# lifeiteng/vall-e

Measured on NVIDIA H100. Metric: audio tokens/sec (AR+NAR d=1024/12L), higher is better.
Workload: dtype bf16

## Files before the change

valle_b200/csrc/attention_wgmma.cu:

```cuda
#include <math_constants.h>

#include "common.cuh"
#include "kernels.cuh"
#include "sm90_ptx.cuh"

namespace vb {
namespace fa3 {

using namespace tc;

constexpr int HD = 64, BQ = 128, BKV = 64;
constexpr int kThreads = 288;
constexpr int kStages = 3;
constexpr int kBoxBytes = 64 * HD * 2;
constexpr int kQBytes = 2 * kBoxBytes;
constexpr int kStageBytes = 2 * kBoxBytes;
constexpr int kSmemBytes = kQBytes + kStages * kStageBytes + 1024  + 256 ;

__device__ __forceinline__ uint64_t make_smem_desc_mn(uint32_t smem_addr) {
  uint64_t d = 0;
  d |= (uint64_t)((smem_addr & 0x3FFFF) >> 4);
  d |= (uint64_t)(1024 >> 4) << 16;
  d |= (uint64_t)(1024 >> 4) << 32;
  d |= (uint64_t)1 << 62;
  return d;
}
__device__ __forceinline__ float ex2(float x) {
  float y;
  asm("ex2.approx.ftz.f32 %0, %1;" : "=f"(y) : "f"(x));
  return y;
}
__device__ __forceinline__ uint32_t pack_bf16(float lo, float hi) {
  __nv_bfloat162 p = __floats2bfloat162_rn(lo, hi);
  return *reinterpret_cast<uint32_t *>(&p);
}

__global__ void __launch_bounds__(kThreads, 2)
attn_wgmma_kernel(const __grid_constant__ CUtensorMap tmap_qkv, int n_head, const int32_t *__restrict__ cu_seqlens,
                  const int32_t *__restrict__ text_lens, const int32_t *__restrict__ seg1_lens, int seg1_start,
                  int mask_mode, bf16 *__restrict__ out, bf16 *__restrict__ kcache, bf16 *__restrict__ vcache,
                  int64_t cache_seq_stride, int cache_cap) {
  const int b = blockIdx.z, h = blockIdx.y;
  const int r0 = cu_seqlens[b], L = cu_seqlens[b + 1] - r0;
  const int q0 = blockIdx.x * BQ;
  if (q0 >= L) return;
  const int S = (mask_mode != VB_MASK_FULL) ? text_lens[b] : 0;
  const int c1 = (mask_mode >= VB_MASK_PADDED_AR) ? seg1_lens[b] : 0;
  const int d = n_head * HD;
  const int q_hi = min(q0 + BQ, L);
  const int kv_max = (mask_mode == VB_MASK_VALLE_AR) ? max(S, q_hi) : L;
  const int n_tiles = (kv_max + BKV - 1) / BKV;

  extern __shared__ uint8_t smem_raw[];
  uint8_t *sq = reinterpret_cast<uint8_t *>((reinterpret_cast<uintptr_t>(smem_raw) + 1023) & ~(uintptr_t)1023);
  uint8_t *ring = sq + kQBytes;
  uint64_t *bars = reinterpret_cast<uint64_t *>(ring + kStages * kStageBytes);
  uint64_t *q_bar = bars, *full_bar = bars + 1, *empty_bar = bars + 1 + kStages;

  const int wg = threadIdx.x >> 7, t = threadIdx.x & 127, lane = threadIdx.x & 31;
  if (threadIdx.x == 0) {
    prefetch_tmap(&tmap_qkv);
    mbar_init(q_bar, 1);
    for (int i = 0; i < kStages; ++i) {
      mbar_init(&full_bar[i], 1);
      mbar_init(&empty_bar[i], 8);
    }
    asm volatile("fence.mbarrier_init.release.cluster;" ::: "memory");
  }
  __syncthreads();

  if (wg == 2) {
    if (t == 0) {
      mbar_expect_tx(q_bar, kQBytes);
      tma_load_2d(&tmap_qkv, q_bar, sq, h * HD, r0 + q0);
      tma_load_2d(&tmap_qkv, q_bar, sq + kBoxBytes, h * HD, r0 + q0 + 64);
      int stage = 0;
      uint32_t phase = 0;
      for (int it = 0; it < n_tiles; ++it) {
        mbar_wait(&empty_bar[stage], phase ^ 1);
        uint8_t *dst = ring + stage * kStageBytes;
        mbar_expect_tx(&full_bar[stage], kStageBytes);
        tma_load_2d(&tmap_qkv, &full_bar[stage], dst, d + h * HD, r0 + it * BKV);
        tma_load_2d(&tmap_qkv, &full_bar[stage], dst + kBoxBytes, 2 * d + h * HD, r0 + it * BKV);
        if (++stage == kStages) {
          stage = 0;
          phase ^= 1;
        }
      }
    }
    return;
  }

  const int half = wg;
  const int row_a = q0 + half * 64 + wg_row(t, 0), row_b = row_a + 8;
  const RowMask lim_a = make_row_mask(mask_mode, row_a, L, S, seg1_start, c1);
  const RowMask lim_b = make_row_mask(mask_mode, row_b, L, S, seg1_start, c1);
  const float sc = 0.125f * 1.4426950408889634f;
  const uint64_t qdesc = make_smem_desc(smem_u32(sq + half * kBoxBytes));

  float o[32];
#pragma unroll
  for (int i = 0; i < 32; ++i) o[i] = 0.f;
  float m_a = -CUDART_INF_F, m_b = -CUDART_INF_F, l_a = 0.f, l_b = 0.f;

  mbar_wait(q_bar, 0);
  int stage = 0;
  uint32_t phase = 0;
  for (int it = 0; it < n_tiles; ++it) {
    const int j0 = it * BKV;
    mbar_wait(&full_bar[stage], phase);
    uint8_t *sk = ring + stage * kStageBytes, *sv = sk + kBoxBytes;
    float s[32];
    const uint64_t kdesc = make_smem_desc(smem_u32(sk));
    wgmma_fence();
#pragma unroll
    for (int k = 0; k < HD / WGMMA_K; ++k) wgmma_m64n64k16(s, qdesc + (uint64_t)(k * 2), kdesc + (uint64_t)(k * 2), k != 0);
    wgmma_commit();
    wgmma_wait<0>();
    wgmma_fence_regs(s);
    if (kcache != nullptr && j0 == q0 + half * 64) {
#pragma unroll
      for (int i = 0; i < 4; ++i) {
        const int idx = t + i * 128;
        const int r = idx >> 3, c = idx & 7;
        if (j0 + r < L) {
          const int64_t off = (int64_t)b * cache_seq_stride + ((int64_t)h * cache_cap + j0 + r) * HD + c * 8;
          const int so = r * 128 + ((c ^ (r & 7)) << 4);
          *reinterpret_cast<uint4 *>(kcache + off) = *reinterpret_cast<const uint4 *>(sk + so);
          *reinterpret_cast<uint4 *>(vcache + off) = *reinterpret_cast<const uint4 *>(sv + so);
        }
      }
    }
    float mx_a = -CUDART_INF_F, mx_b = -CUDART_INF_F;
#pragma unroll
    for (int i = 0; i < 32; ++i) {
      const int c = j0 + wg_col(t, i);
      if ((i >> 1) & 1) {
        s[i] = lim_b.ok(c) ? s[i] * sc : -CUDART_INF_F;
        mx_b = fmaxf(mx_b, s[i]);
      } else {
        s[i] = lim_a.ok(c) ? s[i] * sc : -CUDART_INF_F;
        mx_a = fmaxf(mx_a, s[i]);
      }
    }
    mx_a = fmaxf(mx_a, __shfl_xor_sync(0xffffffffu, mx_a, 1));
    mx_a = fmaxf(mx_a, __shfl_xor_sync(0xffffffffu, mx_a, 2));
    mx_b = fmaxf(mx_b, __shfl_xor_sync(0xffffffffu, mx_b, 1));
    mx_b = fmaxf(mx_b, __shfl_xor_sync(0xffffffffu, mx_b, 2));
    const float mn_a = fmaxf(m_a, mx_a), mn_b = fmaxf(m_b, mx_b);
    const float mu_a = mn_a == -CUDART_INF_F ? 0.f : mn_a, mu_b = mn_b == -CUDART_INF_F ? 0.f : mn_b;
    const float corr_a = ex2(m_a - mu_a), corr_b = ex2(m_b - mu_b);
    m_a = mn_a;
    m_b = mn_b;
    float rs_a = 0.f, rs_b = 0.f;
#pragma unroll
    for (int i = 0; i < 32; ++i) {
      if ((i >> 1) & 1) {
        s[i] = ex2(s[i] - mu_b);
        rs_b += s[i];
        o[i] *= corr_b;
      } else {
        s[i] = ex2(s[i] - mu_a);
        rs_a += s[i];
        o[i] *= corr_a;
      }
    }
    l_a = l_a * corr_a + rs_a;
    l_b = l_b * corr_b + rs_b;
    uint32_t pa[4][4];
#pragma unroll
    for (int ks = 0; ks < 4; ++ks) {
      pa[ks][0] = pack_bf16(s[8 * ks + 0], s[8 * ks + 1]);
      pa[ks][1] = pack_bf16(s[8 * ks + 2], s[8 * ks + 3]);
      pa[ks][2] = pack_bf16(s[8 * ks + 4], s[8 * ks + 5]);
      pa[ks][3] = pack_bf16(s[8 * ks + 6], s[8 * ks + 7]);
    }
    const uint64_t vdesc = make_smem_desc_mn(smem_u32(sv));
    wgmma_fence();
#pragma unroll
    for (int ks = 0; ks < 4; ++ks) wgmma_m64n64k16_rs_tb(o, pa[ks], vdesc + (uint64_t)(ks * (16 * 128 >> 4)));
    wgmma_commit();
    wgmma_wait<0>();
    wgmma_fence_regs(o);
    __syncwarp();
    if (lane == 0) mbar_arrive(&empty_bar[stage]);
    if (++stage == kStages) {
      stage = 0;
      phase ^= 1;
    }
  }
  l_a += __shfl_xor_sync(0xffffffffu, l_a, 1);
  l_a += __shfl_xor_sync(0xffffffffu, l_a, 2);
  l_b += __shfl_xor_sync(0xffffffffu, l_b, 1);
  l_b += __shfl_xor_sync(0xffffffffu, l_b, 2);
  const float inv_a = 1.f / l_a, inv_b = 1.f / l_b;
#pragma unroll
  for (int i = 0; i < 32; i += 2) {
    const bool rb = (i >> 1) & 1;
    const int row = rb ? row_b : row_a;
    if (row >= L) continue;
    const float inv = rb ? inv_b : inv_a;
    *reinterpret_cast<uint32_t *>(out + (int64_t)(r0 + row) * d + h * HD + wg_col(t, i)) =
        pack_bf16(o[i] * inv, o[i + 1] * inv);
  }
}

}

int launch_attention_wgmma(const bf16 *qkv, int64_t M, int B, int n_head, const int32_t *cu_seqlens,
                           const int32_t *text_lens, const int32_t *seg1_lens, int seg1_start, int max_seqlen,
                           int mask_mode, bf16 *out, bf16 *kcache, bf16 *vcache, int64_t cache_seq_stride,
                           int cache_cap, cudaStream_t s) {
  if (M == 0 || B == 0) return VB_OK;
  VB_CHECK_ARG((reinterpret_cast<uintptr_t>(qkv) & 15) == 0, "wgmma attention: qkv must be 16-byte aligned");
  CUtensorMap tm;
  VB_TRY(tc::make_tmap(&tm, qkv, M, 3 * n_head * fa3::HD, 3 * (int64_t)n_head * fa3::HD, 64));
  static PerDeviceOnce once;
  if (once.first())
    VB_CUDA(cudaFuncSetAttribute(fa3::attn_wgmma_kernel, cudaFuncAttributeMaxDynamicSharedMemorySize, fa3::kSmemBytes));
  dim3 grid((max_seqlen + fa3::BQ - 1) / fa3::BQ, n_head, B);
  fa3::attn_wgmma_kernel<<<grid, fa3::kThreads, fa3::kSmemBytes, s>>>(tm, n_head, cu_seqlens, text_lens, seg1_lens,
                                                                      seg1_start, mask_mode, out, kcache, vcache,
                                                                      cache_seq_stride, cache_cap);
  VB_LAUNCH_CHECK();
  return VB_OK;
}

}
```

valle_b200/csrc/sm90_ptx.cuh:

```cuda
#pragma once
#include <cuda.h>

#include <mutex>

#include "common.cuh"

namespace vb {
namespace tc {

constexpr int BK = 64;
constexpr int WGMMA_K = 16;

__device__ __forceinline__ uint32_t smem_u32(const void *p) {
  return static_cast<uint32_t>(__cvta_generic_to_shared(p));
}
__device__ __forceinline__ void mbar_init(uint64_t *bar, uint32_t count) {
  asm volatile("mbarrier.init.shared::cta.b64 [%0], %1;" ::"r"(smem_u32(bar)), "r"(count));
}
__device__ __forceinline__ void mbar_expect_tx(uint64_t *bar, uint32_t bytes) {
  asm volatile("mbarrier.arrive.expect_tx.shared::cta.b64 _, [%0], %1;" ::"r"(smem_u32(bar)), "r"(bytes)
               : "memory");
}
__device__ __forceinline__ void mbar_arrive(uint64_t *bar) {
  asm volatile("mbarrier.arrive.shared::cta.b64 _, [%0];" ::"r"(smem_u32(bar)) : "memory");
}
__device__ __forceinline__ uint32_t mbar_try_wait(uint64_t *bar, uint32_t parity) {
  uint32_t ok;
  asm volatile(
      "{\n"
      ".reg .pred p;\n"
      "mbarrier.try_wait.parity.shared::cta.b64 p, [%1], %2;\n"
      "selp.u32 %0, 1, 0, p;\n"
      "}\n"
      : "=r"(ok)
      : "r"(smem_u32(bar)), "r"(parity)
      : "memory");
  return ok;
}
__device__ __forceinline__ void mbar_wait(uint64_t *bar, uint32_t parity) {
  while (!mbar_try_wait(bar, parity)) {
  }
}
__device__ __forceinline__ void tma_load_2d(const CUtensorMap *map, uint64_t *bar, void *dst, int c0, int c1) {
  asm volatile(
      "cp.async.bulk.tensor.2d.shared::cluster.global.tile.mbarrier::complete_tx::bytes [%0], [%1, {%3, %4}], [%2];"
      ::"r"(smem_u32(dst)), "l"(map), "r"(smem_u32(bar)), "r"(c0), "r"(c1)
      : "memory");
}
__device__ __forceinline__ void prefetch_tmap(const CUtensorMap *map) {
  asm volatile("prefetch.tensormap [%0];" ::"l"(map) : "memory");
}
__device__ __forceinline__ void wgmma_fence() { asm volatile("wgmma.fence.sync.aligned;" ::: "memory"); }
__device__ __forceinline__ void wgmma_commit() { asm volatile("wgmma.commit_group.sync.aligned;" ::: "memory"); }
template <int N> __device__ __forceinline__ void wgmma_wait() {
  asm volatile("wgmma.wait_group.sync.aligned %0;" ::"n"(N) : "memory");
}
template <int R> __device__ __forceinline__ void wgmma_fence_regs(float (&d)[R]) {
#pragma unroll
  for (int i = 0; i < R; ++i) asm volatile("" : "+f"(d[i])::"memory");
}
__device__ __forceinline__ uint64_t make_smem_desc(uint32_t smem_addr) {
  uint64_t d = 0;
  d |= (uint64_t)((smem_addr & 0x3FFFF) >> 4);
  d |= (uint64_t)1 << 16;
  d |= (uint64_t)(1024 >> 4) << 32;
  d |= (uint64_t)1 << 62;
  return d;
}
__device__ __forceinline__ int wg_row(int t, int i) { return ((t >> 5) << 4) + ((t & 31) >> 2) + (((i >> 1) & 1) << 3); }
__device__ __forceinline__ int wg_col(int t, int i) { return ((i >> 2) << 3) + ((t & 3) << 1) + (i & 1); }

__device__ __forceinline__ void wgmma_m64n64k16(float (&d)[32], uint64_t adesc, uint64_t bdesc, uint32_t accumulate) {
  asm volatile(
      "{\n"
      ".reg .pred p;\n"
      "setp.ne.b32 p, %34, 0;\n"
      "wgmma.mma_async.sync.aligned.m64n64k16.f32.bf16.bf16 "
      "{%0, %1, %2, %3, %4, %5, %6, %7, %8, %9, %10, %11, %12, %13, %14, %15, %16, %17, %18, %19, %20, %21, %22, %23, %24, %25, %26, %27, %28, %29, %30, %31}, "
      "%32, %33, p, 1, 1, 0, 0;\n"
      "}\n"
      : "+f"(d[0]), "+f"(d[1]), "+f"(d[2]), "+f"(d[3]), "+f"(d[4]), "+f"(d[5]), "+f"(d[6]), "+f"(d[7]), "+f"(d[8]), "+f"(d[9]), "+f"(d[10]), "+f"(d[11]), "+f"(d[12]), "+f"(d[13]), "+f"(d[14]), "+f"(d[15]), "+f"(d[16]), "+f"(d[17]), "+f"(d[18]), "+f"(d[19]), "+f"(d[20]), "+f"(d[21]), "+f"(d[22]), "+f"(d[23]), "+f"(d[24]), "+f"(d[25]), "+f"(d[26]), "+f"(d[27]), "+f"(d[28]), "+f"(d[29]), "+f"(d[30]), "+f"(d[31])
      : "l"(adesc), "l"(bdesc), "r"(accumulate));
}

__device__ __forceinline__ void wgmma_m64n128k16(float (&d)[64], uint64_t adesc, uint64_t bdesc, uint32_t accumulate) {
  asm volatile(
      "{\n"
      ".reg .pred p;\n"
      "setp.ne.b32 p, %66, 0;\n"
      "wgmma.mma_async.sync.aligned.m64n128k16.f32.bf16.bf16 "
      "{%0, %1, %2, %3, %4, %5, %6, %7, %8, %9, %10, %11, %12, %13, %14, %15, %16, %17, %18, %19, %20, %21, %22, %23, %24, %25, %26, %27, %28, %29, %30, %31, %32, %33, %34, %35, %36, %37, %38, %39, %40, %41, %42, %43, %44, %45, %46, %47, %48, %49, %50, %51, %52, %53, %54, %55, %56, %57, %58, %59, %60, %61, %62, %63}, "
      "%64, %65, p, 1, 1, 0, 0;\n"
      "}\n"
      : "+f"(d[0]), "+f"(d[1]), "+f"(d[2]), "+f"(d[3]), "+f"(d[4]), "+f"(d[5]), "+f"(d[6]), "+f"(d[7]), "+f"(d[8]), "+f"(d[9]), "+f"(d[10]), "+f"(d[11]), "+f"(d[12]), "+f"(d[13]), "+f"(d[14]), "+f"(d[15]), "+f"(d[16]), "+f"(d[17]), "+f"(d[18]), "+f"(d[19]), "+f"(d[20]), "+f"(d[21]), "+f"(d[22]), "+f"(d[23]), "+f"(d[24]), "+f"(d[25]), "+f"(d[26]), "+f"(d[27]), "+f"(d[28]), "+f"(d[29]), "+f"(d[30]), "+f"(d[31]), "+f"(d[32]), "+f"(d[33]), "+f"(d[34]), "+f"(d[35]), "+f"(d[36]), "+f"(d[37]), "+f"(d[38]), "+f"(d[39]), "+f"(d[40]), "+f"(d[41]), "+f"(d[42]), "+f"(d[43]), "+f"(d[44]), "+f"(d[45]), "+f"(d[46]), "+f"(d[47]), "+f"(d[48]), "+f"(d[49]), "+f"(d[50]), "+f"(d[51]), "+f"(d[52]), "+f"(d[53]), "+f"(d[54]), "+f"(d[55]), "+f"(d[56]), "+f"(d[57]), "+f"(d[58]), "+f"(d[59]), "+f"(d[60]), "+f"(d[61]), "+f"(d[62]), "+f"(d[63])
      : "l"(adesc), "l"(bdesc), "r"(accumulate));
}

__device__ __forceinline__ void wgmma_m64n64k16_rs_tb(float (&d)[32], const uint32_t (&a)[4], uint64_t bdesc) {
  asm volatile(
      "{\n"
      ".reg .pred p;\n"
      "setp.ne.b32 p, %37, 0;\n"
      "wgmma.mma_async.sync.aligned.m64n64k16.f32.bf16.bf16 "
      "{%0, %1, %2, %3, %4, %5, %6, %7, %8, %9, %10, %11, %12, %13, %14, %15, %16, %17, %18, %19, %20, %21, %22, %23, %24, %25, %26, %27, %28, %29, %30, %31}, "
      "{%32, %33, %34, %35}, %36, p, 1, 1, 1;\n"
      "}\n"
      : "+f"(d[0]), "+f"(d[1]), "+f"(d[2]), "+f"(d[3]), "+f"(d[4]), "+f"(d[5]), "+f"(d[6]), "+f"(d[7]), "+f"(d[8]), "+f"(d[9]), "+f"(d[10]), "+f"(d[11]), "+f"(d[12]), "+f"(d[13]), "+f"(d[14]), "+f"(d[15]), "+f"(d[16]), "+f"(d[17]), "+f"(d[18]), "+f"(d[19]), "+f"(d[20]), "+f"(d[21]), "+f"(d[22]), "+f"(d[23]), "+f"(d[24]), "+f"(d[25]), "+f"(d[26]), "+f"(d[27]), "+f"(d[28]), "+f"(d[29]), "+f"(d[30]), "+f"(d[31])
      : "r"(a[0]), "r"(a[1]), "r"(a[2]), "r"(a[3]), "l"(bdesc), "r"(1));
}

typedef CUresult (*EncodeTiledFn)(CUtensorMap *, CUtensorMapDataType, cuuint32_t, void *, const cuuint64_t *,
                                  const cuuint64_t *, const cuuint32_t *, const cuuint32_t *,
                                  CUtensorMapInterleave, CUtensorMapSwizzle, CUtensorMapL2promotion,
                                  CUtensorMapFloatOOBfill);

inline EncodeTiledFn get_encode() {
  static EncodeTiledFn fn = nullptr;
  static std::once_flag once;
  std::call_once(once, [] {
    void *p = nullptr;
    cudaDriverEntryPointQueryResult q;
    if (cudaGetDriverEntryPoint("cuTensorMapEncodeTiled", &p, cudaEnableDefault, &q) == cudaSuccess &&
        q == cudaDriverEntryPointSuccess)
      fn = reinterpret_cast<EncodeTiledFn>(p);
  });
  return fn;
}

inline int make_tmap_f32_dense(CUtensorMap *map, const void *ptr, int64_t rows, int64_t cols, int64_t ld, int box_rows,
                               int box_cols) {
  EncodeTiledFn enc = get_encode();
  if (!enc) {
    set_error("tensor map: cuTensorMapEncodeTiled entry point unavailable");
    return VB_ERR_CUDA;
  }
  cuuint64_t dims[2] = {(cuuint64_t)cols, (cuuint64_t)rows};
  cuuint64_t strides[1] = {(cuuint64_t)ld * 4};
  cuuint32_t box[2] = {(cuuint32_t)box_cols, (cuuint32_t)box_rows};
  cuuint32_t estr[2] = {1, 1};
  CUresult r = enc(map, CU_TENSOR_MAP_DATA_TYPE_FLOAT32, 2, const_cast<void *>(ptr), dims, strides, box, estr,
                   CU_TENSOR_MAP_INTERLEAVE_NONE, CU_TENSOR_MAP_SWIZZLE_NONE, CU_TENSOR_MAP_L2_PROMOTION_L2_256B,
                   CU_TENSOR_MAP_FLOAT_OOB_FILL_NONE);
  if (r != CUDA_SUCCESS) {
    set_error("tensor map: cuTensorMapEncodeTiled (fp32 dense) failed (%d) rows=%lld cols=%lld ld=%lld", (int)r,
              (long long)rows, (long long)cols, (long long)ld);
    return VB_ERR_CUDA;
  }
  return VB_OK;
}
inline int make_tmap(CUtensorMap *map, const void *ptr, int64_t rows, int K, int64_t ld, int box_rows) {
  EncodeTiledFn enc = get_encode();
  if (!enc) {
    set_error("wgmma gemm: cuTensorMapEncodeTiled entry point unavailable");
    return VB_ERR_CUDA;
  }
  cuuint64_t dims[2] = {(cuuint64_t)K, (cuuint64_t)rows};
  cuuint64_t strides[1] = {(cuuint64_t)ld * 2};
  cuuint32_t box[2] = {(cuuint32_t)BK, (cuuint32_t)box_rows};
  cuuint32_t estr[2] = {1, 1};
  CUresult r = enc(map, CU_TENSOR_MAP_DATA_TYPE_BFLOAT16, 2, const_cast<void *>(ptr), dims, strides, box, estr,
                   CU_TENSOR_MAP_INTERLEAVE_NONE, CU_TENSOR_MAP_SWIZZLE_128B, CU_TENSOR_MAP_L2_PROMOTION_L2_256B,
                   CU_TENSOR_MAP_FLOAT_OOB_FILL_NONE);
  if (r != CUDA_SUCCESS) {
    set_error("wgmma gemm: cuTensorMapEncodeTiled failed (%d) rows=%lld K=%d ld=%lld", (int)r, (long long)rows, K,
              (long long)ld);
    return VB_ERR_CUDA;
  }
  return VB_OK;
}

}
}
```

Measured before the change: 296,700.

## Restructure FA3 attention kernel with 3 consumer warpgroups and QK/PV overlap

Moves the producer to warpgroup 0 and uses three consumer warpgroups (BQ=192) with setmaxnreg register reallocation, one CTA per SM, and four pipeline stages. It software-pipelines the loop so the next tile's QK^T wgmma is issued alongside the previous tile's PV wgmma, overlapping softmax with tensor-core work. It also skips per-element mask evaluation for tiles that are fully visible. The trade-offs are lower CTA occupancy, larger Q tiles that waste work on short sequences, and more complex barrier and register fencing logic.

```diff
diff --git a/valle_b200/csrc/attention_wgmma.cu b/valle_b200/csrc/attention_wgmma.cu
--- a/valle_b200/csrc/attention_wgmma.cu
+++ b/valle_b200/csrc/attention_wgmma.cu
@@ -9,12 +9,16 @@
 
 using namespace tc;
 
-constexpr int HD = 64, BQ = 128, BKV = 64;
-constexpr int kThreads = 288;
-constexpr int kStages = 3;
+constexpr int HD = 64, BKV = 64;
 constexpr int kBoxBytes = 64 * HD * 2;
-constexpr int kQBytes = 2 * kBoxBytes;
 constexpr int kStageBytes = 2 * kBoxBytes;
+
+constexpr int NWG = 3;
+constexpr int BQ = 64 * NWG;
+constexpr int kThreads = 128 * (NWG + 1);
+constexpr int kStages = 4;
+constexpr int kProdRegs = 24, kConsRegs = 160;
+constexpr int kQBytes = NWG * kBoxBytes;
 constexpr int kSmemBytes = kQBytes + kStages * kStageBytes + 1024  + 256 ;
 
 __device__ __forceinline__ uint64_t make_smem_desc_mn(uint32_t smem_addr) {
@@ -34,8 +38,67 @@
   __nv_bfloat162 p = __floats2bfloat162_rn(lo, hi);
   return *reinterpret_cast<uint32_t *>(&p);
 }
-
-__global__ void __launch_bounds__(kThreads, 2)
+template <int R> __device__ __forceinline__ void fence_u32(uint32_t (&a)[R][4]) {
+#pragma unroll
+  for (int i = 0; i < R; ++i)
+#pragma unroll
+    for (int k = 0; k < 4; ++k) asm volatile("" : "+r"(a[i][k])::"memory");
+}
+
+__device__ __forceinline__ void issue_qk(float (&s)[32], uint64_t qdesc, const uint8_t *sk) {
+  const uint64_t kdesc = make_smem_desc(smem_u32(sk));
+#pragma unroll
+  for (int k = 0; k < HD / WGMMA_K; ++k) wgmma_m64n64k16(s, qdesc + (uint64_t)(k * 2), kdesc + (uint64_t)(k * 2), k != 0);
+}
+__device__ __forceinline__ void issue_pv(float (&o)[32], const uint32_t (&pa)[4][4], const uint8_t *sv) {
+  const uint64_t vdesc = make_smem_desc_mn(smem_u32(sv));
+#pragma unroll
+  for (int ks = 0; ks < 4; ++ks) wgmma_m64n64k16_rs_tb(o, pa[ks], vdesc + (uint64_t)(ks * (16 * 128 >> 4)));
+}
+
+template <bool MASKED>
+__device__ __forceinline__ void softmax_block(float (&s)[32], int j0, int t, const RowMask &lim_a, const RowMask &lim_b,
+                                              float &m_a, float &m_b, float &l_a, float &l_b, float &corr_a,
+                                              float &corr_b) {
+  const float sc = 0.125f * 1.4426950408889634f;
+  float mx_a = -CUDART_INF_F, mx_b = -CUDART_INF_F;
+#pragma unroll
+  for (int i = 0; i < 32; ++i) {
+    const int c = j0 + wg_col(t, i);
+    if ((i >> 1) & 1) {
+      s[i] = (!MASKED || lim_b.ok(c)) ? __fmul_rn(s[i], sc) : -CUDART_INF_F;
+      mx_b = fmaxf(mx_b, s[i]);
+    } else {
+      s[i] = (!MASKED || lim_a.ok(c)) ? __fmul_rn(s[i], sc) : -CUDART_INF_F;
+      mx_a = fmaxf(mx_a, s[i]);
+    }
+  }
+  mx_a = fmaxf(mx_a, __shfl_xor_sync(0xffffffffu, mx_a, 1));
+  mx_a = fmaxf(mx_a, __shfl_xor_sync(0xffffffffu, mx_a, 2));
+  mx_b = fmaxf(mx_b, __shfl_xor_sync(0xffffffffu, mx_b, 1));
+  mx_b = fmaxf(mx_b, __shfl_xor_sync(0xffffffffu, mx_b, 2));
+  const float mn_a = fmaxf(m_a, mx_a), mn_b = fmaxf(m_b, mx_b);
+  const float mu_a = mn_a == -CUDART_INF_F ? 0.f : mn_a, mu_b = mn_b == -CUDART_INF_F ? 0.f : mn_b;
+  corr_a = ex2(m_a - mu_a);
+  corr_b = ex2(m_b - mu_b);
+  m_a = mn_a;
+  m_b = mn_b;
+  float rs_a = 0.f, rs_b = 0.f;
+#pragma unroll
+  for (int i = 0; i < 32; ++i) {
+    if ((i >> 1) & 1) {
+      s[i] = ex2(s[i] - mu_b);
+      rs_b += s[i];
+    } else {
+      s[i] = ex2(s[i] - mu_a);
+      rs_a += s[i];
+    }
+  }
+  l_a = l_a * corr_a + rs_a;
+  l_b = l_b * corr_b + rs_b;
+}
+
+__global__ void __launch_bounds__(kThreads, 1)
 attn_wgmma_kernel(const __grid_constant__ CUtensorMap tmap_qkv, int n_head, const int32_t *__restrict__ cu_seqlens,
                   const int32_t *__restrict__ text_lens, const int32_t *__restrict__ seg1_lens, int seg1_start,
                   int mask_mode, bf16 *__restrict__ out, bf16 *__restrict__ kcache, bf16 *__restrict__ vcache,
@@ -44,6 +107,7 @@
   const int r0 = cu_seqlens[b], L = cu_seqlens[b + 1] - r0;
   const int q0 = blockIdx.x * BQ;
   if (q0 >= L) return;
+  const int n_wg = min(NWG, (L - q0 + 63) >> 6);
   const int S = (mask_mode != VB_MASK_FULL) ? text_lens[b] : 0;
   const int c1 = (mask_mode >= VB_MASK_PADDED_AR) ? seg1_lens[b] : 0;
   const int d = n_head * HD;
@@ -63,17 +127,17 @@
     mbar_init(q_bar, 1);
     for (int i = 0; i < kStages; ++i) {
       mbar_init(&full_bar[i], 1);
-      mbar_init(&empty_bar[i], 8);
+      mbar_init(&empty_bar[i], 4 * n_wg);
     }
     asm volatile("fence.mbarrier_init.release.cluster;" ::: "memory");
   }
   __syncthreads();
 
-  if (wg == 2) {
+  if (wg == 0) {
+    setmaxnreg_dec<kProdRegs>();
     if (t == 0) {
-      mbar_expect_tx(q_bar, kQBytes);
-      tma_load_2d(&tmap_qkv, q_bar, sq, h * HD, r0 + q0);
-      tma_load_2d(&tmap_qkv, q_bar, sq + kBoxBytes, h * HD, r0 + q0 + 64);
+      mbar_expect_tx(q_bar, n_wg * kBoxBytes);
+      for (int w = 0; w < n_wg; ++w) tma_load_2d(&tmap_qkv, q_bar, sq + w * kBoxBytes, h * HD, r0 + q0 + 64 * w);
       int stage = 0;
       uint32_t phase = 0;
       for (int it = 0; it < n_tiles; ++it) {
@@ -90,35 +154,25 @@
     }
     return;
   }
-
-  const int half = wg;
-  const int row_a = q0 + half * 64 + wg_row(t, 0), row_b = row_a + 8;
+  setmaxnreg_inc<kConsRegs>();
+
+  const int w = wg - 1;
+  if (w >= n_wg) return;
+  const int row_a = q0 + w * 64 + wg_row(t, 0), row_b = row_a + 8;
   const RowMask lim_a = make_row_mask(mask_mode, row_a, L, S, seg1_start, c1);
   const RowMask lim_b = make_row_mask(mask_mode, row_b, L, S, seg1_start, c1);
-  const float sc = 0.125f * 1.4426950408889634f;
-  const uint64_t qdesc = make_smem_desc(smem_u32(sq + half * kBoxBytes));
+  const uint64_t qdesc = make_smem_desc(smem_u32(sq + w * kBoxBytes));
 
   float o[32];
 #pragma unroll
   for (int i = 0; i < 32; ++i) o[i] = 0.f;
   float m_a = -CUDART_INF_F, m_b = -CUDART_INF_F, l_a = 0.f, l_b = 0.f;
-
-  mbar_wait(q_bar, 0);
-  int stage = 0;
-  uint32_t phase = 0;
-  for (int it = 0; it < n_tiles; ++it) {
-    const int j0 = it * BKV;
-    mbar_wait(&full_bar[stage], phase);
-    uint8_t *sk = ring + stage * kStageBytes, *sv = sk + kBoxBytes;
-    float s[32];
-    const uint64_t kdesc = make_smem_desc(smem_u32(sk));
-    wgmma_fence();
-#pragma unroll
-    for (int k = 0; k < HD / WGMMA_K; ++k) wgmma_m64n64k16(s, qdesc + (uint64_t)(k * 2), kdesc + (uint64_t)(k * 2), k != 0);
-    wgmma_commit();
-    wgmma_wait<0>();
-    wgmma_fence_regs(s);
-    if (kcache != nullptr && j0 == q0 + half * 64) {
+  float s[32];
+  uint32_t pa[4][4];
+
+  auto softmax_step = [&](int j0, const uint8_t *sk, float &corr_a, float &corr_b) {
+    if (kcache != nullptr && j0 == q0 + w * 64) {
+      const uint8_t *sv = sk + kBoxBytes;
 #pragma unroll
       for (int i = 0; i < 4; ++i) {
         const int idx = t + i * 128;
@@ -131,43 +185,16 @@
         }
       }
     }
-    float mx_a = -CUDART_INF_F, mx_b = -CUDART_INF_F;
-#pragma unroll
-    for (int i = 0; i < 32; ++i) {
-      const int c = j0 + wg_col(t, i);
-      if ((i >> 1) & 1) {
-        s[i] = lim_b.ok(c) ? s[i] * sc : -CUDART_INF_F;
-        mx_b = fmaxf(mx_b, s[i]);
-      } else {
-        s[i] = lim_a.ok(c) ? s[i] * sc : -CUDART_INF_F;
-        mx_a = fmaxf(mx_a, s[i]);
-      }
-    }
-    mx_a = fmaxf(mx_a, __shfl_xor_sync(0xffffffffu, mx_a, 1));
-    mx_a = fmaxf(mx_a, __shfl_xor_sync(0xffffffffu, mx_a, 2));
-    mx_b = fmaxf(mx_b, __shfl_xor_sync(0xffffffffu, mx_b, 1));
-    mx_b = fmaxf(mx_b, __shfl_xor_sync(0xffffffffu, mx_b, 2));
-    const float mn_a = fmaxf(m_a, mx_a), mn_b = fmaxf(m_b, mx_b);
-    const float mu_a = mn_a == -CUDART_INF_F ? 0.f : mn_a, mu_b = mn_b == -CUDART_INF_F ? 0.f : mn_b;
-    const float corr_a = ex2(m_a - mu_a), corr_b = ex2(m_b - mu_b);
-    m_a = mn_a;
-    m_b = mn_b;
-    float rs_a = 0.f, rs_b = 0.f;
-#pragma unroll
-    for (int i = 0; i < 32; ++i) {
-      if ((i >> 1) & 1) {
-        s[i] = ex2(s[i] - mu_b);
-        rs_b += s[i];
-        o[i] *= corr_b;
-      } else {
-        s[i] = ex2(s[i] - mu_a);
-        rs_a += s[i];
-        o[i] *= corr_a;
-      }
-    }
-    l_a = l_a * corr_a + rs_a;
-    l_b = l_b * corr_b + rs_b;
-    uint32_t pa[4][4];
+    const bool seen_a = j0 + BKV <= lim_a.lim0 || (j0 >= lim_a.s1 && j0 + BKV <= lim_a.hi1);
+    const bool seen_b = j0 + BKV <= lim_b.lim0 || (j0 >= lim_b.s1 && j0 + BKV <= lim_b.hi1);
+    if (__all_sync(0xffffffffu, seen_a && seen_b))
+      softmax_block<false>(s, j0, t, lim_a, lim_b, m_a, m_b, l_a, l_b, corr_a, corr_b);
+    else
+      softmax_block<true>(s, j0, t, lim_a, lim_b, m_a, m_b, l_a, l_b, corr_a, corr_b);
+  };
+  auto rescale_pack = [&](float corr_a, float corr_b) {
+#pragma unroll
+    for (int i = 0; i < 32; ++i) o[i] *= ((i >> 1) & 1) ? corr_b : corr_a;
 #pragma unroll
     for (int ks = 0; ks < 4; ++ks) {
       pa[ks][0] = pack_bf16(s[8 * ks + 0], s[8 * ks + 1]);
@@ -175,20 +202,54 @@
       pa[ks][2] = pack_bf16(s[8 * ks + 4], s[8 * ks + 5]);
       pa[ks][3] = pack_bf16(s[8 * ks + 6], s[8 * ks + 7]);
     }
-    const uint64_t vdesc = make_smem_desc_mn(smem_u32(sv));
-    wgmma_fence();
-#pragma unroll
-    for (int ks = 0; ks < 4; ++ks) wgmma_m64n64k16_rs_tb(o, pa[ks], vdesc + (uint64_t)(ks * (16 * 128 >> 4)));
+  };
+  auto release = [&](int st) {
+    wgmma_fence_regs(o);
+    fence_u32(pa);
+    __syncwarp();
+    if (lane == 0) mbar_arrive(&empty_bar[st]);
+  };
+
+  mbar_wait(q_bar, 0);
+  mbar_wait(&full_bar[0], 0);
+  wgmma_fence();
+  issue_qk(s, qdesc, ring);
+  wgmma_commit();
+  wgmma_wait<0>();
+  wgmma_fence_regs(s);
+  {
+    float corr_a, corr_b;
+    softmax_step(0, ring, corr_a, corr_b);
+    rescale_pack(corr_a, corr_b);
+  }
+  int prev = 0, stage = 1;
+  uint32_t phase = 0;
+  for (int it = 1; it < n_tiles; ++it) {
+    uint8_t *sk = ring + stage * kStageBytes;
+    mbar_wait(&full_bar[stage], phase);
+      wgmma_fence();
+    issue_qk(s, qdesc, sk);
     wgmma_commit();
+    issue_pv(o, pa, ring + prev * kStageBytes + kBoxBytes);
+    wgmma_commit();
+      wgmma_wait<1>();
+    wgmma_fence_regs(s);
+    float corr_a, corr_b;
+    softmax_step(it * BKV, sk, corr_a, corr_b);
     wgmma_wait<0>();
-    wgmma_fence_regs(o);
-    __syncwarp();
-    if (lane == 0) mbar_arrive(&empty_bar[stage]);
+    release(prev);
+    rescale_pack(corr_a, corr_b);
+    prev = stage;
     if (++stage == kStages) {
       stage = 0;
       phase ^= 1;
     }
   }
+  wgmma_fence();
+  issue_pv(o, pa, ring + prev * kStageBytes + kBoxBytes);
+  wgmma_commit();
+  wgmma_wait<0>();
+  release(prev);
   l_a += __shfl_xor_sync(0xffffffffu, l_a, 1);
   l_a += __shfl_xor_sync(0xffffffffu, l_a, 2);
   l_b += __shfl_xor_sync(0xffffffffu, l_b, 1);
diff --git a/valle_b200/csrc/sm90_ptx.cuh b/valle_b200/csrc/sm90_ptx.cuh
--- a/valle_b200/csrc/sm90_ptx.cuh
+++ b/valle_b200/csrc/sm90_ptx.cuh
@@ -49,6 +49,12 @@
 }
 __device__ __forceinline__ void prefetch_tmap(const CUtensorMap *map) {
   asm volatile("prefetch.tensormap [%0];" ::"l"(map) : "memory");
+}
+template <int N> __device__ __forceinline__ void setmaxnreg_dec() {
+  asm volatile("setmaxnreg.dec.sync.aligned.u32 %0;" ::"n"(N));
+}
+template <int N> __device__ __forceinline__ void setmaxnreg_inc() {
+  asm volatile("setmaxnreg.inc.sync.aligned.u32 %0;" ::"n"(N));
 }
 __device__ __forceinline__ void wgmma_fence() { asm volatile("wgmma.fence.sync.aligned;" ::: "memory"); }
 __device__ __forceinline__ void wgmma_commit() { asm volatile("wgmma.commit_group.sync.aligned;" ::: "memory"); }
```

New measurement: 304,700 (median of 6 runs). +2.7%, better.
